# drepion43/distributed-mnist-BNNs

Measured on AMD Instinct MI355X. Metric: train samples/sec (node) + binary GEMM TOPS, higher is better.
Workload: dtype fp4/fp6/int8 MFMA (ternary operands as FP4 e2m1, fp32 operands as 4 FP6 e2m3 digit planes with E8M0 block scales + an FP4 residual plane on the dX operands (backward: within 2^-19 / 2^-22 of the block maximum) or 3 int8 digit planes (first layer); fp32 accumulate, fp32 I/O); 1 GPU; wide binarized MLP 784-8192x3-10 (BASELINE config 5); model=wide, global_batch=65536, per_gpu_batch=65536, seq_len=1, parallelism=dp1, backend=fp4, exchange=False, hip_graph=False

## Files before the change

distributed-mnist-bnns_amd/bnn_amd/functional.py:

```python
import collections
import contextlib
import ctypes
import itertools
import os

import torch

from . import _lib as L

__all__ = [
    "KernelTimer", "timing", "sign", "sign_pack", "sign_pack_bits", "quant_rows", "quant_cols_t", "gemm_i8", "gemm_xnor",
    "quant6_rows", "quant6_cols_t", "gemm_fp6", "set_digit_gemm",
    "binary_linear", "binary_conv2d", "hardtanh_backward", "adam_clamp_", "adam_clamp_pack_", "packed_weight",
    "sgd_clamp_", "sgd_clamp_multi_", "sgd_clamp_pack_",
    "invalidate_packed", "batch_norm_hardtanh",
    "bn_hardtanh_binary_linear", "batch_norm2d_hardtanh_pool", "dropout_batch_norm_hardtanh", "dropout_mask",
    "BinaryLinearFunction", "BinaryConv2dFunction",
]

ALIGN = 64


class KernelTimer:

# ... 879 lines not shown

def _const_vec(val, n, device):
    key = (float(val), int(n), str(device))
    t = _CONST.get(key)
    if t is None:
        t = torch.full((n,), float(val), dtype=torch.float32, device=device)
        _CONST[key] = t
    return t


PIX_STATS = os.environ.get("BNN_PIX_STATS", "1") != "0"
_FSTATS_ATTR = "_bnn_fstats"
PIX_STATS_USES = 0


def _pixels_fwd_with_stats(q, wq, M, N, K, bscale, bias, R, s0):
    chunk = int(L.lib().bnn_gemm_i8_bnstats_chunk(M, N))
    rows = (M + chunk - 1) // chunk
    part = torch.empty((2, rows, N), dtype=torch.float64, device=q.device)
    y = torch.empty((M, N), dtype=torch.float32, device=q.device)
    Kp = q.shape[1]
    assert wq.shape[1] == Kp and Kp % ALIGN == 0
    name = f"{gemm_kernel_name(1, 1, M, N, Kp)} [pixels]" if _TIMER is not None else ""
    with _timed(name, 2.0 * M * N * K, M * Kp + N * Kp + 4 * M * N):
        L.call("bnn_gemm_i8_affine_bnstats", q, Kp, wq, Kp, bscale, bias, R, float(s0), y, N, M, N, Kp, part, rows,
               L.stream())
    setattr(y, _FSTATS_ATTR, (part, rows, chunk, M, N, "pixels", 0.0, 0))
    return y


S20 = os.environ.get("BNN_S20", "1") != "0"
S20_HANDOFFS = 0


def _s20_of(x):
    z = getattr(x, _PREACT_ATTR, None)
    return z.args if z is not None and z.kind == "s20" else None


def dense_preact(z):
    d = getattr(z, _PREACT_ATTR, None)
    return z if d is None else d.dense()


def _pixels_fwd_s20(q, wq, M, N, K, a, bias, R, s0):
    chunk = int(L.lib().bnn_gemm_i8_bnstats_chunk(M, N))
    rows = (M + chunk - 1) // chunk
    dev = q.device
    part = torch.empty((2, rows, N), dtype=torch.float64, device=dev)
    lo = torch.empty((M, N), dtype=torch.int16, device=dev)
    hi = torch.empty((M, N // 2), dtype=torch.uint8, device=dev)
    Kp = q.shape[1]
    assert wq.shape[1] == Kp and Kp % ALIGN == 0
    name = f"{gemm_kernel_name(1, 1, M, N, Kp)} [pixels s20]" if _TIMER is not None else ""
    with _timed(name, 2.0 * M * N * K, M * Kp + N * Kp + 2.5 * M * N):
        L.call("bnn_gemm_i8_affine_bnstats_s20", q, Kp, wq, Kp, R, float(s0), K, lo, hi, N, M, N, Kp, part, rows,
               _const_vec(a, N, dev), bias, L.stream())
    y = _preact_carrier(PreAct("s20", lo, hi, bias, float(a)))
    setattr(y, _FSTATS_ATTR, (part, rows, chunk, M, N, "pixels", 0.0, 0))
    return y


def _fstats_of(z, M, C, drop=(0.0, 0)):
    fs = getattr(z, _FSTATS_ATTR, None)
    if fs is None or fs[3] != M or fs[4] != C or z._version != 0:
        return None
    p, seed = float(drop[0]), int(drop[1])
    if fs[6] != p or (p > 0 and fs[7] != seed):
        return None
    return fs


FP4_STATS = os.environ.get("BNN_FP4_STATS", "1") != "0"
FP4_STATS_USES = 0


def _fp4_fwd_with_stats(q, wq, M, N, k_true, bias, zbias, chunk, i16, drop=(0.0, 0)):
    Kb = q.shape[1]
    assert wq.shape[1] == Kb and Kb % ALIGN == 0
    rows = (M + chunk - 1) // chunk
    part = torch.empty((2, rows, N), dtype=torch.float64, device=q.device)
    C = torch.empty((M, N), dtype=torch.int16 if i16 else torch.float32, device=q.device)
    name = (gemm_kernel_name(0, 0, M, N, Kb) + (" [i16]" if i16 else "")) if _TIMER is not None else ""
    with _timed(name, 2.0 * M * N * k_true, (M + N) * Kb + (2 if i16 else 4) * M * N):
        L.call("bnn_gemm_fp4_bnstats", q, Kb, wq, Kb, None if i16 else bias, None if i16 else C, C if i16 else None, N,
               zbias, M, N, Kb, float(drop[0]), int(drop[1]), part, rows, L.stream())
    return C, (part, rows, chunk, M, N, "fp4", float(drop[0]), int(drop[1]))


class BinaryLinearPixelsFunction(torch.autograd.Function):

    @staticmethod
    def forward(ctx, u, weight, bias, a, s0, cache=False, emit_s20=False):
        _check(u, dtype=torch.uint8)
        _check(weight, bias)
        M, K = u.shape
        N = weight.shape[0]
        ctx.dims = (M, K, N)
        ctx.has_bias = bias is not None
        ctx.a, ctx.s0 = a, s0
        need_dw = ctx.needs_input_grad[1]
        q, qt = pixels_pack(u, want_q=M > 0, want_qt=need_dw and M > 0)
        if M == 0:
            ctx.save_for_backward(None)
            return torch.empty((0, N), dtype=torch.float32, device=u.device)
        wq, _ = packed_weight(weight, "i8", True, False, cache)
        R = row_sums(wq, K)
# ... 173 lines not shown
        L.call("bnn_hinge_bwd", x, y, t, M, C, float(margin), int(bool(squared)), go, dx, L.stream())
    return dx


def hinge_loss_ok(input, target):
    if not (torch.is_tensor(input) and torch.is_tensor(target) and input.is_cuda and input.dim() == 2
            and input.dtype == torch.float32 and input.shape[0] > 0 and target.device == input.device
            and bool(L.lib().bnn_hinge_ok(input.shape[1]))):
        return False
    if target.dtype == torch.int64:
        return target.dim() == 1 and target.shape[0] == input.shape[0]
    return target.dtype == torch.float32 and target.shape == input.shape and not target.requires_grad


def hinge_loss(input, target, margin=1.0, squared=False):
    _check(input)
    if not hinge_loss_ok(input, target):
        raise ValueError("bnn_amd: hinge_loss needs float32 CUDA [M, C] logits (M > 0, C in 2, 10, 16, 32, 64) and "
                         f"int64 [M] labels or a float32 target of the same shape without grad; got "
                         f"{tuple(input.shape)} {input.dtype} and {tuple(target.shape)} {target.dtype}")
    return HingeLossFunction.apply(input, target, float(margin), bool(squared))


def _pair_same(v, what):
    if isinstance(v, (tuple, list)):
        if len(set(v)) != 1:
            raise NotImplementedError(f"bnn_amd: asymmetric {what} {v} is not supported")
        return int(v[0])
    return int(v)


C1BN = os.environ.get("BNN_C1BN", "1") != "0"
_C1BN_WANT = "_bnn_c1bn_consumer"
_C1BN_ATTR = "_bnn_c1bn"
C1BN_HANDOFFS = 0


_C1bnHandoff = collections.namedtuple("_C1bnHandoff", "zq zb zf dyp mean invstd gw gb sg sgx inv_n ht")


def _c1bn_take(dy):
    ent = _take(dy, _C1BN_ATTR, stale="stale conv1 / BatchNorm2d hand-off",
                lost="a conv gradient placeholder lost its BatchNorm2d hand-off")
    return None if ent is None else _C1bnHandoff(*ent)


_CONV_C1F = [os.environ.get("BNN_CONV_C1F")]
if os.environ.get("BNN_FP6_PERS") is not None:
    L.call("bnn_gemm_fp6_set_persistent", int(os.environ["BNN_FP6_PERS"] != "0"))
if os.environ.get("BNN_FP6_HALF") is not None:
    L.call("bnn_gemm_fp6_set_half", int(os.environ["BNN_FP6_HALF"]), 0.0)
if os.environ.get("BNN_PIX_TILE") is not None:
    L.call("bnn_gemm_i8_bnstats_set_tile", int(os.environ["BNN_PIX_TILE"]))
if os.environ.get("BNN_HEAD_RED_COLS") is not None:
    L.call("bnn_bn_set_head_reduce_cols", int(os.environ["BNN_HEAD_RED_COLS"]))


def _conv_env():
    if _CONV_C1F[0] is not None:
        L.call("bnn_conv_set_c1_filter", int(_CONV_C1F[0] != "0"))
        _CONV_C1F[0] = None


ZQ = True
ZQ_HANDOFFS = 0


def _zq_fmt(x, binarize_input, stride, dilation, groups, C, KH, KW, H, W, pad, N, Co):
    if not (ZQ and binarize_input and stride == 1 and dilation == 1 and groups == 1 and pad <= min(KH, KW) - 1):
        return 0
    if not (C == 1 and KW <= 8) and not (C % 16 == 0 and C <= 64):
        return 0
    fmt = 2 if C * KH * KW <= 32767 else 0
    if fmt and not L.lib().bnn_conv2d_fwd_q_ok(fmt, N, C, H, W, Co, KH, KW, stride, pad, dilation, groups):
        return 0
    return fmt


def conv_out_hw(H, W, KH, KW, stride, padding, dilation):
    eh, ew = dilation * (KH - 1) + 1, dilation * (KW - 1) + 1
    if eh > H + 2 * padding or ew > W + 2 * padding:
        raise ValueError(f"conv2d: dilated kernel ({eh} x {ew}) can't be greater than the padded input "
                         f"({H + 2 * padding} x {W + 2 * padding})")
    return (H + 2 * padding - eh) // stride + 1, (W + 2 * padding - ew) // stride + 1


class BinaryConv2dFunction(torch.autograd.Function):
    @staticmethod
    def forward(ctx, x, weight, bias, binarize_input, stride, padding, dilation, groups, emit_compact=False,
                stochastic=None):
        _check(x, weight, bias)
        OH, OW = conv_out_hw(x.shape[2], x.shape[3], weight.shape[2], weight.shape[3], stride, padding, dilation)
        _conv_env()
        x = _c2d(x)
        if stochastic is not None and binarize_input:
            x = binarize_stochastic(x, stochastic)
        w = _c2d(weight.detach())
        N, C, H, W = x.shape
        Co, _, KH, KW = w.shape
        b = bias.detach() if bias is not None else None
        ctx.empty = N == 0
        ctx.save_for_backward(x, w)
        ctx.conf = (binarize_input, stride, padding, dilation, groups)
        ctx.has_bias = bias is not None
        zf = _zq_fmt(x, binarize_input, stride, dilation, groups, C, KH, KW, H, W, padding, N, Co) if emit_compact else 0
        if zf and N > 0 and Co <= 64 and (OH * OW) % 4 == 0 and OH % 2 == 0 and OW % 2 == 0:
# ... 867 lines not shown
```

distributed-mnist-bnns_amd/csrc/bnn_gemm.hip:

```cpp
#include <algorithm>
#include <type_traits>

#include "bnn_common.h"

namespace bnn {
namespace {

constexpr int BK = 64;

struct GemmParams {
  const int8_t* A;
  const int8_t* B;
  int64_t lda, ldb, a_plane, b_plane;
  const float* a_scale;
  const float* b_scale;
  const float* bias;
  float* C;
  int64_t ldc;
  int M, N, K;
  int gm, gn;
  const int64_t* row_off;
  const int64_t* col_off;
  double off_mul;
  int16_t* C16 = nullptr;
// ... 718 lines not shown
            const uint32_t lo = (uint32_t)(uint16_t)(int16_t)v.x | ((uint32_t)(uint16_t)(int16_t)v.y << 16);
            const uint32_t hi = (uint32_t)(uint16_t)(int16_t)v.z | ((uint32_t)(uint16_t)(int16_t)v.w << 16);
            out_store2u(d16, lo, hi);
          } else {
            const float vs[4] = {v.x, v.y, v.z, v.w};
#pragma unroll
            for (int j = 0; j < 4; ++j)
              if (c0 + j < p.N) d16[j] = (int16_t)vs[j];
          }
          continue;
        }
        float* dst = p.C + (int64_t)row * p.ldc + c0;
#ifdef GEMM_DIAG_NOSTORE
        if (p.M > 0) continue;
#endif
        if (vec_ok && c0 + 3 < p.N) {
          out_store4f(dst, v);
        } else {
          const float vs[4] = {v.x, v.y, v.z, v.w};
#pragma unroll
          for (int j = 0; j < 4; ++j)
            if (c0 + j < p.N) dst[j] = vs[j];
        }
      }
      asm volatile("s_waitcnt lgkmcnt(0)" ::: "memory");
    }
  }
}

template <int DA, int DB, int WAVES_M, int WAVES_N, int WM, int WN, int STAGES, int BKT, int IL = 0,
          int DIAG = 0, int S16 = 0, int BST = 0>
__global__ __launch_bounds__(64 * WAVES_M * WAVES_N) void gemm_i8_v2_k(GemmParams p) {
  gemm_v2_body<DA, DB, WAVES_M, WAVES_N, WM, WN, STAGES, BKT, IL, DIAG, 0, S16, BST>(p);
}

template <int WAVES_M, int WAVES_N, int WM, int WN, int STAGES, int BKT, int IL = 0, int S16 = 0, int BST = 0>
__global__ __launch_bounds__(64 * WAVES_M * WAVES_N) void gemm_fp4_k(GemmParams p) {
  gemm_v2_body<1, 1, WAVES_M, WAVES_N, WM, WN, STAGES, BKT, IL, 0, 1, S16, BST>(p);
}

template <int WAVES_M, int WAVES_N, int WM, int WN, int STAGES, int BKT, int IL = 0, int S16 = 0, int BST = 0>
__global__ __launch_bounds__(64 * WAVES_M * WAVES_N, 2) void gemm_fp4_h_k(GemmParams p) {
  gemm_v2_body<1, 1, WAVES_M, WAVES_N, WM, WN, STAGES, BKT, IL, 0, 1, S16, BST>(p);
}

template <int WAVES_M, int WAVES_N, int WM, int WN, int STAGES, int BKT, int IL = 0, int S16 = 0>
__global__ __launch_bounds__(64 * WAVES_M * WAVES_N) void gemm_fp4_bnsign_k(GemmParams p) {
  gemm_v2_body<1, 1, WAVES_M, WAVES_N, WM, WN, STAGES, BKT, IL, 0, 1, S16, 0, 1>(p);
}

template <int WAVES_M, int WAVES_N, int WM, int WN, int STAGES, int BKT>
__global__ __launch_bounds__(64 * WAVES_M * WAVES_N) void gemm_i8_bnsign_k(GemmParams p) {
  gemm_v2_body<1, 1, WAVES_M, WAVES_N, WM, WN, STAGES, BKT, 0, 0, 0, 0, 0, 1>(p);
}

template <int F4, int WAVES_M, int WAVES_N, int WM, int WN, int STAGES, int BKT, int IL = 0, int S16 = 0>
int launch_bnsign(GemmParams p, hipStream_t s) {
  constexpr int BM = WAVES_M * WM * 32, BN = WAVES_N * WN * 32;
  p.gm = (p.M + BM - 1) / BM;
  p.gn = (p.N + BN - 1) / BN;
  const int64_t covered = (int64_t)p.gn * BN / 2;
  if (covered < p.ldq4) {
    const hipError_t e = hipMemset2DAsync(p.Q4 + covered, (size_t)p.ldq4, 0, (size_t)(p.ldq4 - covered), (size_t)p.M, s);
    if (e != hipSuccess) {
      set_error("bnn_gemm_bnsign: clearing the pad failed: %s", hipGetErrorString(e));
      return (int)e;
    }
  }
  const dim3 grid((unsigned)((int64_t)p.gm * p.gn)), block(64 * WAVES_M * WAVES_N);
  if constexpr (F4) {
    hipLaunchKernelGGL((gemm_fp4_bnsign_k<WAVES_M, WAVES_N, WM, WN, STAGES, BKT, IL, S16>), grid, block, 0, s, p);
    return check_launch("bnn_gemm_fp4_bnsign");
  } else {
    static_assert(IL == 0 && S16 == 0, "int8 BN-sign form: the 32x32 BK=64 kernels");
    hipLaunchKernelGGL((gemm_i8_bnsign_k<WAVES_M, WAVES_N, WM, WN, STAGES, BKT>), grid, block, 0, s, p);
    return check_launch("bnn_gemm_i8_affine_bnsign");
  }
}

template <int WAVES_M, int WAVES_N, int WM, int WN, int STAGES, int BKT, int IL = 0, int S16 = 0, int BST = 0>
int launch_fp4h(GemmParams p, hipStream_t s) {
  constexpr int BM = WAVES_M * WM * 32, BN = WAVES_N * WN * 32;
  p.gm = (p.M + BM - 1) / BM;
  p.gn = (p.N + BN - 1) / BN;
  hipLaunchKernelGGL((gemm_fp4_h_k<WAVES_M, WAVES_N, WM, WN, STAGES, BKT, IL, S16, BST>),
                     dim3((unsigned)((int64_t)p.gm * p.gn)), dim3(64 * WAVES_M * WAVES_N), 0, s, p);
  return check_launch("bnn_gemm_fp4");
}

template <int DA, int DB, int WAVES_M, int WAVES_N, int WM, int WN, int STAGES, int BKT, int IL = 0,
          int DIAG = 0, int F4 = 0, int S16 = 0, int BST = 0>
int launch_v2(GemmParams p, hipStream_t s) {
  constexpr int BM = WAVES_M * WM * 32, BN = WAVES_N * WN * 32;
  p.gm = (p.M + BM - 1) / BM;
  p.gn = (p.N + BN - 1) / BN;
  const int64_t nblk = (int64_t)p.gm * p.gn;
  if constexpr (F4) {
    static_assert(DA == 1 && DB == 1 && DIAG == 0, "FP4 form");
    hipLaunchKernelGGL((gemm_fp4_k<WAVES_M, WAVES_N, WM, WN, STAGES, BKT, IL, S16, BST>), dim3((unsigned)nblk),
                       dim3(64 * WAVES_M * WAVES_N), 0, s, p);
    return check_launch("bnn_gemm_fp4");
  } else {
    hipLaunchKernelGGL((gemm_i8_v2_k<DA, DB, WAVES_M, WAVES_N, WM, WN, STAGES, BKT, IL, DIAG, S16, BST>),
                       dim3((unsigned)nblk), dim3(64 * WAVES_M * WAVES_N), 0, s, p);
    return check_launch("bnn_gemm_i8");
  }
// ... 80 lines not shown
    id = base + g_variant;
    alt = base + 1;
  } else if (a_digits == 1) {
    const bool big = ((M + 255) / 256) * ((N + 255) / 256) >= 512;
    id = big ? 9 : 1;
    alt = big ? 2 : 1;
  } else if (b_digits == 1) {
    const bool big = ((M + 127) / 128) * ((N + 255) / 256) >= 256;
    id = big ? 18 : 13;
    alt = big ? 15 : 13;
  } else {
    id = 22;
    alt = 22;
  }
  const Variant* v = find_variant(id);
  if (v == nullptr) v = find_variant(base + 1);
  if (K % v->bk != 0) v = find_variant(alt);
  return v;
}

}
}

using namespace bnn;

BNN_API int bnn_gemm_i8_affine(const int8_t* A, int64_t lda, int64_t a_plane, int32_t a_digits,
                               const int8_t* B, int64_t ldb, int64_t b_plane, int32_t b_digits,
                               const float* a_scale, const float* b_scale, const float* bias,
                               const int64_t* row_off, const int64_t* col_off, double off_mul, float* C,
                               int64_t ldc, int64_t M, int64_t N, int64_t K, void* stream) {
  const bool cfg_ok = (a_digits == 1 && b_digits == 1) || (a_digits == 3 && b_digits == 1) ||
                      (a_digits == 3 && b_digits == 3);
  if (!A || !B || !C || !cfg_ok || M < 0 || N < 0 || K <= 0 || K % BK != 0 || lda < K || ldb < K ||
      lda % 16 != 0 || ldb % 16 != 0 || ldc < N || !aligned16(A) || !aligned16(B) ||
      M > 0x7fffffff || N > 0x7fffffff || K > 0x7fffffff ||
      (a_digits > 1 && (a_plane < M * lda || a_plane % 16 != 0)) ||
      (b_digits > 1 && (b_plane < N * ldb || b_plane % 16 != 0))) {
    set_error("bnn_gemm_i8_affine: bad arguments (M=%lld N=%lld K=%lld lda=%lld ldb=%lld digits=%d,%d; "
              "K must be a positive multiple of 64)",
              (long long)M, (long long)N, (long long)K, (long long)lda, (long long)ldb, a_digits,
              b_digits);
    return kErrInval;
  }
  if (M == 0 || N == 0) return 0;
  GemmParams p{A, B, lda, ldb, a_plane, b_plane, a_scale, b_scale, bias, C, ldc,
               (int)M, (int)N, (int)K, 0, 0, row_off, col_off, off_mul};
  p.raster = g_raster;
  if (lda * 256 >= (1LL << 31) || ldb * 256 >= (1LL << 31))
    return find_variant(a_digits == 1 ? 0 : (b_digits == 1 ? 10 : 20))->fn(p, reinterpret_cast<hipStream_t>(stream));
  return pick_kernel(a_digits, b_digits, M, N, K)->fn(p, reinterpret_cast<hipStream_t>(stream));
}

static int g_i8_bnstats_tile = 0;

static const Variant* i8_bnstats_variant(int64_t M, int64_t N) {
  const bool big = ((M + 255) / 256) * ((N + 255) / 256) >= 512;
  if (g_i8_bnstats_tile != 0) return find_variant(g_i8_bnstats_tile == 2 ? 2 : 1);
  return find_variant(big ? 2 : 1);
}

BNN_API int32_t bnn_gemm_i8_bnstats_set_tile(int32_t tile) {
  if (tile < 0) return g_i8_bnstats_tile;
  if (tile > 2) return kErrInval;
  g_i8_bnstats_tile = tile;
  return 0;
}

BNN_API int64_t bnn_gemm_i8_bnstats_chunk(int64_t M, int64_t N) {
  return i8_bnstats_variant(M, N)->id == 2 ? 128 : 64;
}

static bool i8_bnstats_shape_ok(int64_t M, int64_t N, int64_t K, int64_t lda, int64_t ldb) {
  return M > 0 && N > 0 && K > 0 && K % BK == 0 && lda >= K && ldb >= K && lda % 16 == 0 && ldb % 16 == 0 &&
         M <= 0x7fffffff && N <= 0x7fffffff && K <= 0x7fffffff && lda * 256 < (1LL << 31) &&
         ldb * 256 < (1LL << 31) &&
         (double)M * (128.0 * K) * (128.0 * K) < 9007199254740992.0;
}

BNN_API int bnn_gemm_i8_bnstats_ok(int64_t M, int64_t N, int64_t K, int64_t lda, int64_t ldb) {
  return i8_bnstats_shape_ok(M, N, K, lda, ldb) ? 1 : 0;
}

BNN_API int bnn_gemm_i8_affine_bnstats(const int8_t* A, int64_t lda, const int8_t* B, int64_t ldb,
                                       const float* b_scale, const float* bias, const int64_t* col_off,
                                       double off_mul, float* C, int64_t ldc, int64_t M, int64_t N, int64_t K,
                                       double* stat, int64_t stat_rows, void* stream) {
  const int64_t chunk = M > 0 ? bnn_gemm_i8_bnstats_chunk(M, N) : 1;
  if (!A || !B || !C || !stat || !i8_bnstats_shape_ok(M, N, K, lda, ldb) || ldc < N || !aligned16(A) ||
      !aligned16(B) || stat_rows != (M + chunk - 1) / chunk) {
    set_error("bnn_gemm_i8_affine_bnstats: bad arguments (M=%lld N=%lld K=%lld stat_rows=%lld; want %lld)",
              (long long)M, (long long)N, (long long)K, (long long)stat_rows, (long long)((M + chunk - 1) / chunk));
    return kErrInval;
  }
  GemmParams p{A, B, lda, ldb, 0, 0, nullptr, b_scale, bias, C, ldc,
               (int)M, (int)N, (int)K, 0, 0, nullptr, col_off, off_mul};
  p.stat = stat;
  p.stat_rows = stat_rows;
  hipStream_t st = reinterpret_cast<hipStream_t>(stream);
  return i8_bnstats_variant(M, N)->id == 2 ? launch_v2<1, 1, 2, 4, 4, 2, 3, 64, 0, 0, 0, 0, 1>(p, st)
                                           : launch_v2<1, 1, 2, 2, 2, 2, 3, 64, 0, 0, 0, 0, 1>(p, st);
}

BNN_API int bnn_gemm_i8_s20_ok(int64_t M, int64_t N, int64_t K, int64_t k_true, double s0) {
  return (N % 4 == 0 && s0 == (double)(int64_t)s0 && k_true > 0 && k_true <= K &&
          (double)k_true * (128.0 + fabs(s0)) < 524288.0)
             ? 1
             : 0;
}

BNN_API int bnn_gemm_i8_affine_bnstats_s20(const int8_t* A, int64_t lda, const int8_t* B, int64_t ldb,
                                           const int64_t* col_off, double off_mul, int64_t k_true, int16_t* Slo,
                                           uint8_t* Shi, int64_t ldc, int64_t M, int64_t N, int64_t K, double* stat,
                                           int64_t stat_rows, const float* b_scale, const float* bias, void* stream) {
  const int64_t chunk = M > 0 ? bnn_gemm_i8_bnstats_chunk(M, N) : 1;
  if (!A || !B || !Slo || !Shi || !col_off || !stat || !i8_bnstats_shape_ok(M, N, K, lda, ldb) || ldc < N ||
      ldc % 4 != 0 || !aligned16(A) || !aligned16(B) || (reinterpret_cast<uintptr_t>(Slo) & 7) != 0 ||
      (reinterpret_cast<uintptr_t>(Shi) & 1) != 0 || !bnn_gemm_i8_s20_ok(M, N, K, k_true, off_mul) ||
      stat_rows != (M + chunk - 1) / chunk) {
    set_error("bnn_gemm_i8_affine_bnstats_s20: bad arguments (M=%lld N=%lld K=%lld k_true=%lld off_mul=%g "
              "stat_rows=%lld)", (long long)M, (long long)N, (long long)K, (long long)k_true, off_mul,
              (long long)stat_rows);
    return kErrInval;
  }
  GemmParams p{A, B, lda, ldb, 0, 0, nullptr, b_scale, bias, nullptr, ldc,
               (int)M, (int)N, (int)K, 0, 0, nullptr, col_off, off_mul};
  p.stat = stat;
  p.stat_rows = stat_rows;
  p.S20lo = Slo;
  p.S20hi = Shi;
  hipStream_t st = reinterpret_cast<hipStream_t>(stream);
  return i8_bnstats_variant(M, N)->id == 2 ? launch_v2<1, 1, 2, 4, 4, 2, 3, 64, 0, 0, 0, 0, 1>(p, st)
                                           : launch_v2<1, 1, 2, 2, 2, 2, 3, 64, 0, 0, 0, 0, 1>(p, st);
}

BNN_API int bnn_gemm_i8(const int8_t* A, int64_t lda, int64_t a_plane, int32_t a_digits,
                        const int8_t* B, int64_t ldb, int64_t b_plane, int32_t b_digits,
                        const float* a_scale, const float* b_scale, const float* bias, float* C,
                        int64_t ldc, int64_t M, int64_t N, int64_t K, void* stream) {
  return bnn_gemm_i8_affine(A, lda, a_plane, a_digits, B, ldb, b_plane, b_digits, a_scale, b_scale, bias,
                            nullptr, nullptr, 0.0, C, ldc, M, N, K, stream);
}

BNN_API int bnn_gemm_fp4(const uint8_t* A, int64_t lda, const uint8_t* B, int64_t ldb, const float* bias,
                         float* C, int64_t ldc, int64_t M, int64_t N, int64_t K, void* stream) {
  if (!A || !B || !C || M < 0 || N < 0 || K <= 0 || K % BK != 0 || lda < K || ldb < K || lda % 16 != 0 ||
      ldb % 16 != 0 || ldc < N || !aligned16(A) || !aligned16(B) || M > 0x7fffffff || N > 0x7fffffff ||
      K > 0x7fffffff || lda * 256 >= (1LL << 31) || ldb * 256 >= (1LL << 31)) {
    set_error("bnn_gemm_fp4: bad arguments (M=%lld N=%lld K=%lld bytes; K must be a positive multiple of 64 "
              "and below 2^23 bytes)",
              (long long)M, (long long)N, (long long)K);
    return kErrInval;
  }
  if (M == 0 || N == 0) return 0;
  GemmParams p{reinterpret_cast<const int8_t*>(A), reinterpret_cast<const int8_t*>(B), lda, ldb, 0, 0,
               nullptr, nullptr, bias, C, ldc, (int)M, (int)N, (int)K, 0, 0, nullptr, nullptr, 0.0};
  return pick_kernel(0, 0, M, N, K)->fn(p, reinterpret_cast<hipStream_t>(stream));
}

BNN_API int bnn_gemm_fp4_i16(const uint8_t* A, int64_t lda, const uint8_t* B, int64_t ldb, int16_t* C16,
                             int64_t ldc, int64_t M, int64_t N, int64_t K, void* stream) {
  if (!C16 || ldc % 4 != 0 || (reinterpret_cast<uintptr_t>(C16) & 7) != 0 || 2 * K > 32767) {
    set_error("bnn_gemm_fp4_i16: bad arguments (ldc=%lld, K=%lld bytes; ldc %% 4 == 0, 8-B aligned output, "
              "2K <= 32767)", (long long)ldc, (long long)K);
    return kErrInval;
  }
  if (!A || !B || M < 0 || N < 0 || K <= 0 || K % BK != 0 || lda < K || ldb < K || lda % 16 != 0 ||
      ldb % 16 != 0 || ldc < N || !aligned16(A) || !aligned16(B) || M > 0x7fffffff || N > 0x7fffffff ||
      lda * 256 >= (1LL << 31) || ldb * 256 >= (1LL << 31)) {
    set_error("bnn_gemm_fp4_i16: bad arguments (M=%lld N=%lld K=%lld bytes)", (long long)M, (long long)N,
              (long long)K);
    return kErrInval;
  }
  if (M == 0 || N == 0) return 0;
  GemmParams p{reinterpret_cast<const int8_t*>(A), reinterpret_cast<const int8_t*>(B), lda, ldb, 0, 0,
               nullptr, nullptr, nullptr, nullptr, ldc, (int)M, (int)N, (int)K, 0, 0, nullptr, nullptr, 0.0, C16};
  return pick_kernel(0, 0, M, N, K)->fn(p, reinterpret_cast<hipStream_t>(stream));
}

BNN_API int64_t bnn_gemm_fp4_bnstats_chunk(int64_t M, int64_t N, int64_t K) {
  const int id = pick_kernel(0, 0, M, N, K)->id;
  return id == 31 ? 64 : (id == 36 ? 128 : 0);
}

BNN_API int bnn_gemm_fp4_bnstats(const uint8_t* A, int64_t lda, const uint8_t* B, int64_t ldb, const float* bias,
                                 float* C, int16_t* C16, int64_t ldc, const float* zbias, int64_t M, int64_t N,
// ... 94 lines not shown
```

include/bnn.h:

```cpp
#ifndef BNN_H_
#define BNN_H_

#include <stdint.h>

#ifdef __cplusplus
extern "C" {
#endif

#define BNN_EINVAL (-1)

typedef void* bnn_stream_t;

int bnn_version(void);
const char* bnn_last_error(void);

int bnn_sign_pack_i8(const float* x, int64_t M, int64_t K, int64_t ldx, int8_t* q, int64_t ldq,
                     int8_t* qt, int64_t ldqt, bnn_stream_t stream);

int bnn_sign_pack_fp4(const float* x, int64_t M, int64_t K, int64_t ldx, uint8_t* q4, int64_t ldq4,
                      int8_t* qt, int64_t ldqt, int32_t qt_fmt, bnn_stream_t stream);

int bnn_sign_f32(const float* x, float* y, int64_t n, bnn_stream_t stream);

int bnn_sign_pack_fp4_out(const float* x, int64_t M, int64_t K, uint8_t* q4, int64_t ldq4, int8_t* qt,
                          int64_t ldqt, int32_t qt_fmt, float* sout, bnn_stream_t stream);

int bnn_binarize_stoch_f32(const float* x, float* y, int64_t n, uint64_t seed, bnn_stream_t stream);
int bnn_stoch_pack_i8(const float* x, int64_t M, int64_t K, int64_t ldx, int8_t* q, int64_t ldq, int8_t* qt,
                      int64_t ldqt, uint64_t seed, bnn_stream_t stream);
int bnn_stoch_pack_fp4(const float* x, int64_t M, int64_t K, int64_t ldx, uint8_t* q4, int64_t ldq4, int8_t* qt,
                       int64_t ldqt, int32_t qt_fmt, uint64_t seed, int32_t force, bnn_stream_t stream);
int bnn_stoch_pack_fp4_out(const float* x, int64_t M, int64_t K, uint8_t* q4, int64_t ldq4, int8_t* qt,
                           int64_t ldqt, int32_t qt_fmt, float* sout, uint64_t seed, int32_t force,
                           bnn_stream_t stream);

int bnn_sign_pack_bits(const float* x, int64_t M, int64_t K, int64_t ldx, uint32_t* sbits,
                       uint32_t* nzbits, int64_t ldw, bnn_stream_t stream);

int bnn_quant_rows(const float* x, int64_t M, int64_t K, int64_t ldx, int8_t* digits, int64_t ldq,
                   int64_t plane, float* scale, bnn_stream_t stream);

int64_t bnn_quant_cols_workspace(int64_t M, int64_t N);
int bnn_quant_cols_t(const float* x, int64_t M, int64_t N, int64_t ldx, int8_t* digits_t,
                     int64_t ldqt, int64_t plane, float* scale, float* colsum, void* work,
                     bnn_stream_t stream);
int bnn_quant_cols_t_dsum(const float* x, int64_t M, int64_t N, int64_t ldx, int8_t* digits_t,
                          int64_t ldqt, int64_t plane, float* scale, float* colsum, int64_t* dsum,
                          void* work, bnn_stream_t stream);

int bnn_gemm_i8(const int8_t* A, int64_t lda, int64_t a_plane, int32_t a_digits,
                const int8_t* B, int64_t ldb, int64_t b_plane, int32_t b_digits,
                const float* a_scale, const float* b_scale, const float* bias, float* C,
                int64_t ldc, int64_t M, int64_t N, int64_t K, bnn_stream_t stream);

int bnn_gemm_i8_affine(const int8_t* A, int64_t lda, int64_t a_plane, int32_t a_digits,
                       const int8_t* B, int64_t ldb, int64_t b_plane, int32_t b_digits,
                       const float* a_scale, const float* b_scale, const float* bias,
                       const int64_t* row_off, const int64_t* col_off, double off_mul, float* C,
                       int64_t ldc, int64_t M, int64_t N, int64_t K, bnn_stream_t stream);

int64_t bnn_gemm_i8_bnstats_chunk(int64_t M, int64_t N);

int64_t bnn_gemm_fp4_bnstats_chunk(int64_t M, int64_t N, int64_t K);
int bnn_gemm_fp4_bnstats(const uint8_t* A, int64_t lda, const uint8_t* B, int64_t ldb, const float* bias,
                         float* C, int16_t* C16, int64_t ldc, const float* zbias, int64_t M, int64_t N, int64_t K,
                         float drop_p, uint64_t drop_seed, double* stat, int64_t stat_rows, bnn_stream_t stream);
int bnn_gemm_i8_bnstats_set_tile(int32_t tile);
int bnn_gemm_i8_affine_bnstats(const int8_t* A, int64_t lda, const int8_t* B, int64_t ldb,
                               const float* b_scale, const float* bias, const int64_t* col_off,
                               double off_mul, float* C, int64_t ldc, int64_t M, int64_t N, int64_t K,
                               double* stat, int64_t stat_rows, bnn_stream_t stream);
int bnn_gemm_i8_bnstats_ok(int64_t M, int64_t N, int64_t K, int64_t lda, int64_t ldb);

int bnn_gemm_i8_s20_ok(int64_t M, int64_t N, int64_t K, int64_t k_true, double s0);
int bnn_gemm_i8_affine_bnstats_s20(const int8_t* A, int64_t lda, const int8_t* B, int64_t ldb,
                                   const int64_t* col_off, double off_mul, int64_t k_true, int16_t* Slo,
                                   uint8_t* Shi, int64_t ldc, int64_t M, int64_t N, int64_t K, double* stat,
                                   int64_t stat_rows, const float* b_scale, const float* bias, bnn_stream_t stream);

int bnn_unit_to_pixels(const float* x, int64_t n, uint8_t* u, int32_t* bad, bnn_stream_t stream);
int bnn_pixels_pack(const uint8_t* x, int64_t M, int64_t K, int64_t ldx, int8_t* q, int64_t ldq,
                    int8_t* qt, int64_t ldqt, bnn_stream_t stream);
int bnn_row_sums(const int8_t* q, int64_t N, int64_t K, int64_t ldq, int64_t* out, bnn_stream_t stream);

int bnn_gemm_fp4(const uint8_t* A, int64_t lda, const uint8_t* B, int64_t ldb, const float* bias,
                 float* C, int64_t ldc, int64_t M, int64_t N, int64_t K, bnn_stream_t stream);

int bnn_gemm_fp4_i16(const uint8_t* A, int64_t lda, const uint8_t* B, int64_t ldb, int16_t* C16, int64_t ldc,
                     int64_t M, int64_t N, int64_t K, bnn_stream_t stream);

int bnn_gemm_fp4_bnsign(const uint8_t* A, int64_t lda, const uint8_t* B, int64_t ldb, const float* bias,
                        const float* mean, const float* invstd, const float* gamma, const float* beta,
                        uint8_t* q4, int64_t ldq4, int64_t M, int64_t N, int64_t K, bnn_stream_t stream);
int bnn_gemm_i8_affine_bnsign(const int8_t* A, int64_t lda, const int8_t* B, int64_t ldb,
                              const float* b_scale, const float* bias, const int64_t* col_off, double off_mul,
                              const float* mean, const float* invstd, const float* gamma, const float* beta,
                              uint8_t* q4, int64_t ldq4, int64_t M, int64_t N, int64_t K, bnn_stream_t stream);

int bnn_gemm_set_variant(int32_t variant);
int bnn_gemm_set_raster(int32_t raster);
const char* bnn_gemm_i8_kernel(int32_t a_digits, int32_t b_digits, int64_t M, int64_t N,
                               int64_t K);

int64_t bnn_quant6_scale_rows(int64_t rows);
int bnn_quant6_rows(const float* x, int64_t M, int64_t K, int64_t ldx, int64_t Kp, uint8_t* lo, uint8_t* hi,
                    uint8_t* sc, uint8_t* res , bnn_stream_t stream);
int64_t bnn_quant6_cols_workspace(int64_t M, int64_t N);
int bnn_quant6_cols_t(const float* x, int64_t M, int64_t N, int64_t ldx, int64_t Mp, uint8_t* lo, uint8_t* hi,
                      uint8_t* sc, float* colsum, void* work, bnn_stream_t stream);
int bnn_gemm_fp6(const uint8_t* alo, const uint8_t* ahi, const uint8_t* asc, int64_t asc_rows, const uint8_t* ares,
                 const uint8_t* b, int64_t ldb, const float* bias, float* C, int64_t ldc, int64_t M, int64_t N,
                 int64_t K, bnn_stream_t stream);
int64_t bnn_gemm_fp6_workspace(int64_t M, int64_t N, int64_t K);
int bnn_gemm_fp6_ws(const uint8_t* alo, const uint8_t* ahi, const uint8_t* asc, int64_t asc_rows,
                    const uint8_t* ares, const uint8_t* b, int64_t ldb, const float* bias, float* C, int64_t ldc,
                    int64_t M, int64_t N, int64_t K, void* work, int64_t work_bytes, bnn_stream_t stream);
int64_t bnn_fp4_panel_bytes(int64_t N, int64_t Kp);
int bnn_fp4_panelize(const uint8_t* b, int64_t N, int64_t ldb, int64_t Kp, uint8_t* panels, bnn_stream_t stream);
int bnn_gemm_fp6_panel_ws(const uint8_t* alo, const uint8_t* ahi, const uint8_t* asc, int64_t asc_rows,
                          const uint8_t* ares, const uint8_t* bpanels, int64_t bks, const float* bias, float* C,
                          int64_t ldc, int64_t M, int64_t N, int64_t K, void* work, int64_t work_bytes,
                          bnn_stream_t stream);
int64_t bnn_gemm_fp6_bnstats_rows(int64_t M);
int bnn_gemm_fp6_bnstats(const uint8_t* alo, const uint8_t* ahi, const uint8_t* asc, int64_t asc_rows,
                         const uint8_t* ares, const uint8_t* bpanels, int64_t bks, float* C, int64_t ldc, int64_t M,
                         int64_t N, int64_t K,
                         const void* x, const float* xbias, int32_t x_i16, const float* mean, const float* mean_lo,
// ... 299 lines not shown
```

Before: 1.528 million samples/s.

## Add dedicated u8-pixel s20 first-layer GEMM kernel with LDS-patch packed epilogue

Adds a specialized int8 MFMA kernel for the first-layer pixel GEMM that writes the split 20-bit output (int16 low plane plus 4-bit high nibbles). The epilogue stages accumulators through a swizzled LDS patch, packs them, and uses DPP lane moves so each row segment goes out as wide 16-byte stores. It also fuses the BN statistics reduction. The new default (form 2) runs a smaller one-wave-row tile with 2 stages and occupancy 3, replacing the generic v2 kernel for large shapes. This adds code complexity and changes tile shape and occupancy, which may or may not suit the MI355X.

```diff
diff --git a/distributed-mnist-bnns_amd/bnn_amd/functional.py b/distributed-mnist-bnns_amd/bnn_amd/functional.py
--- a/distributed-mnist-bnns_amd/bnn_amd/functional.py
+++ b/distributed-mnist-bnns_amd/bnn_amd/functional.py
@@ -955,7 +955,7 @@
     hi = torch.empty((M, N // 2), dtype=torch.uint8, device=dev)
     Kp = q.shape[1]
     assert wq.shape[1] == Kp and Kp % ALIGN == 0
-    name = f"{gemm_kernel_name(1, 1, M, N, Kp)} [pixels s20]" if _TIMER is not None else ""
+    name = f"{L.lib().bnn_gemm_i8_s20_kernel(M, N).decode()} [pixels s20]" if _TIMER is not None else ""
     with _timed(name, 2.0 * M * N * K, M * Kp + N * Kp + 2.5 * M * N):
         L.call("bnn_gemm_i8_affine_bnstats_s20", q, Kp, wq, Kp, R, float(s0), K, lo, hi, N, M, N, Kp, part, rows,
                _const_vec(a, N, dev), bias, L.stream())
@@ -1235,6 +1235,8 @@
     L.call("bnn_gemm_fp6_set_half", int(os.environ["BNN_FP6_HALF"]), 0.0)
 if os.environ.get("BNN_PIX_TILE") is not None:
     L.call("bnn_gemm_i8_bnstats_set_tile", int(os.environ["BNN_PIX_TILE"]))
+if os.environ.get("BNN_PIX_S20_FORM") is not None:
+    L.call("bnn_gemm_i8_s20_set_form", int(os.environ["BNN_PIX_S20_FORM"]))
 if os.environ.get("BNN_HEAD_RED_COLS") is not None:
     L.call("bnn_bn_set_head_reduce_cols", int(os.environ["BNN_HEAD_RED_COLS"]))
 
diff --git a/distributed-mnist-bnns_amd/csrc/bnn_gemm.hip b/distributed-mnist-bnns_amd/csrc/bnn_gemm.hip
--- a/distributed-mnist-bnns_amd/csrc/bnn_gemm.hip
+++ b/distributed-mnist-bnns_amd/csrc/bnn_gemm.hip
@@ -794,6 +794,194 @@
 template <int WAVES_M, int WAVES_N, int WM, int WN, int STAGES, int BKT>
 __global__ __launch_bounds__(64 * WAVES_M * WAVES_N) void gemm_i8_bnsign_k(GemmParams p) {
   gemm_v2_body<1, 1, WAVES_M, WAVES_N, WM, WN, STAGES, BKT, 0, 0, 0, 0, 0, 1>(p);
+}
+
+__device__ __forceinline__ void out_store4u(void* p, uint32_t a, uint32_t b, uint32_t c, uint32_t d) {
+  if (BNN_NT_STORES) __builtin_nontemporal_store(v4u{a, b, c, d}, reinterpret_cast<v4u*>(p));
+  else *reinterpret_cast<uint4*>(p) = make_uint4(a, b, c, d);
+}
+
+template <int DA, int DB, int WAVES_M, int WAVES_N, int WM, int WN, int STAGES, int BKT, int OCC = 2>
+__global__ __launch_bounds__(64 * WAVES_M * WAVES_N, OCC) void gemm_i8_px_s20_k(GemmParams p) {
+  static_assert(DA == 1 && DB == 1 && WN == 2 && BKT == 64, "the u8-pixel (1,1) form, patch pairs, BK = 64");
+  constexpr int NW = WAVES_M * WAVES_N;
+  constexpr int BM = WAVES_M * WM * 32, BN = WAVES_N * WN * 32;
+  constexpr int A_ST = BM * BKT, B_ST = BN * BKT, ST = A_ST + B_ST;
+  constexpr int RPI = 1024 / BKT, CPR = BKT / 16;
+  constexpr int IA = BM / RPI, IB = BN / RPI;
+  static_assert(IA % NW == 0 && IB % NW == 0, "glds instructions must split evenly over waves");
+  constexpr int PER_WAVE = (IA + IB) / NW;
+  constexpr int KSTEPS = BKT / 32;
+  constexpr int PATCH = 32 * 64;
+  static_assert(NW * PATCH * 4 <= STAGES * ST, "the epilogue's patches reuse the operand ring");
+  __shared__ __attribute__((aligned(16))) char smem[STAGES * ST];
+
+  const int lane = threadIdx.x & 63, wave = wave_id();
+  const int wm = wave / WAVES_N, wn = wave % WAVES_N;
+  int tm, tn;
+  tile_of(blockIdx.x, p.gm, p.gn, tm, tn);
+  const int m0 = tm * BM, n0 = tn * BN;
+
+  auto swz = [](int row) { return (row >> 2) & 3; };
+  const int srow = lane / CPR, sslot = lane % CPR;
+  const int lim_a = p.M - 1 - m0, lim_b = p.N - 1 - n0;
+  auto stage = [&](int kt, int buf) {
+    char* sA = smem + buf * ST;
+    char* sB = sA + A_ST;
+#pragma unroll
+    for (int i = 0; i < IA / NW; ++i) {
+      const int jr = wave + i * NW;
+      const int lrow = jr * RPI + srow;
+      const uint32_t voff = (uint32_t)min(lrow, lim_a) * (uint32_t)p.lda + 16u * (uint32_t)(sslot ^ swz(lrow));
+      glds16_s(p.A + (int64_t)m0 * p.lda + (int64_t)kt * BKT, voff, sA + jr * 1024);
+    }
+#pragma unroll
+    for (int i = 0; i < IB / NW; ++i) {
+      const int jr = wave + i * NW;
+      const int lrow = jr * RPI + srow;
+      const uint32_t voff = (uint32_t)min(lrow, lim_b) * (uint32_t)p.ldb + 16u * (uint32_t)(sslot ^ swz(lrow));
+      glds16_s(p.B + (int64_t)n0 * p.ldb + (int64_t)kt * BKT, voff, sB + jr * 1024);
+    }
+  };
+
+  v16i acc[WM][WN];
+#pragma unroll
+  for (int t = 0; t < WM; ++t)
+#pragma unroll
+    for (int u = 0; u < WN; ++u) acc[t][u] = v16i{0};
+
+  const int r = lane & 31, h = lane >> 5, sw = swz(r);
+  const int nk = p.K / BKT;
+#pragma unroll
+  for (int s = 0; s < STAGES - 1; ++s)
+    if (s < nk) stage(s, s);
+  for (int kt = 0; kt < nk; ++kt) {
+    wait_stages<PER_WAVE, STAGES - 2>(min(STAGES - 2, nk - 1 - kt));
+    block_barrier();
+    if (kt + STAGES - 1 < nk) stage(kt + STAGES - 1, (kt + STAGES - 1) % STAGES);
+    const char* sA = smem + (kt % STAGES) * ST;
+    const char* sB = sA + A_ST;
+    v4i a[2][WM], b[2][WN];
+    auto load_frags = [&](int ks, v4i (&fa)[WM], v4i (&fb)[WN]) {
+      const int off = 16 * ((2 * ks + h) ^ sw);
+#pragma unroll
+      for (int t = 0; t < WM; ++t)
+        fa[t] = *reinterpret_cast<const v4i*>(sA + (wm * WM * 32 + t * 32 + r) * BKT + off);
+#pragma unroll
+      for (int u = 0; u < WN; ++u)
+        fb[u] = *reinterpret_cast<const v4i*>(sB + (wn * WN * 32 + u * 32 + r) * BKT + off);
+    };
+    load_frags(0, a[0], b[0]);
+#pragma unroll
+    for (int ks = 0; ks < KSTEPS; ++ks) {
+      if (ks + 1 < KSTEPS) load_frags(ks + 1, a[(ks + 1) & 1], b[(ks + 1) & 1]);
+#pragma unroll
+      for (int t = 0; t < WM; ++t)
+#pragma unroll
+        for (int u = 0; u < WN; ++u)
+          acc[t][u] = __builtin_amdgcn_mfma_i32_32x32x32_i8(a[ks & 1][t], b[ks & 1][u], acc[t][u], 0, 0, 0);
+    }
+  }
+  wait_vmcnt_c<0>();
+  block_barrier();
+
+  const int cr0 = m0 + wm * WM * 32;
+  const int cnt = min(WM * 32, p.M - cr0);
+  const bool full = cr0 + WM * 32 <= p.M;
+  const int lim = p.M - cr0 - 4 * h;
+  const int64_t chunk = (int64_t)tm * WAVES_M + wm, RN = p.stat_rows * (int64_t)p.N;
+  int icoff[WN];
+#pragma unroll
+  for (int u = 0; u < WN; ++u) {
+    const int col = n0 + wn * WN * 32 + u * 32 + r;
+    const bool cin = col < p.N;
+    const double coff = cin ? (double)p.col_off[col] * p.off_mul : 0.0;
+    icoff[u] = (int)coff;
+    int i1 = 0;
+    double d2 = 0.0;
+#pragma unroll
+    for (int t = 0; t < WM; ++t)
+#pragma unroll
+      for (int i = 0; i < 16; ++i) {
+        const int v = (full || (t * 32 + (i & 3) + 8 * (i >> 2)) < lim) ? acc[t][u][i] : 0;
+        const double d = (double)v;
+        i1 += v;
+        d2 = fma(d, d, d2);
+      }
+    i1 += __shfl_xor(i1, 32, 64);
+    d2 += __shfl_xor(d2, 32, 64);
+    if (h == 0 && cnt > 0 && cin) {
+      const double s1 = (double)i1, s2 = d2;
+      const double a = p.b_scale ? (double)p.b_scale[col] : 1.0;
+      const double b = p.bias ? (double)p.bias[col] : 0.0;
+      p.stat[chunk * p.N + col] = a * (s1 + cnt * coff) + cnt * b;
+      const double m2 = s2 - s1 * s1 / cnt;
+      p.stat[RN + chunk * p.N + col] = a * a * (m2 > 0.0 ? m2 : 0.0);
+    }
+  }
+
+  int* patch = reinterpret_cast<int*>(smem) + wave * PATCH;
+  const int tcol0 = n0 + wn * WN * 32;
+  const int lc8 = lane & 7;
+  const int c0 = tcol0 + 8 * lc8;
+  const bool lo16 = ((p.ldc & 7) == 0) && ((reinterpret_cast<uintptr_t>(p.S20lo) & 15) == 0);
+  const bool hi16 = ((p.ldc & 31) == 0) && ((reinterpret_cast<uintptr_t>(p.S20hi) & 15) == 0) &&
+                    tcol0 + 32 * (lc8 >> 2) + 32 <= p.N;
+#pragma unroll
+  for (int t = 0; t < WM; ++t) {
+    const int trow0 = m0 + wm * WM * 32 + t * 32;
+#pragma unroll
+    for (int u = 0; u < WN; ++u)
+#pragma unroll
+      for (int i = 0; i < 16; ++i) {
+        const int lr = (i & 3) + 8 * (i >> 2) + 4 * h;
+        const int lc = u * 32 + r;
+        patch[lr * 64 + ((((lc >> 2) ^ (i & 1)) << 2) | (lc & 3))] = acc[t][u][i] + icoff[u];
+      }
+    asm volatile("s_waitcnt lgkmcnt(0)" ::: "memory");
+#pragma unroll
+    for (int ps = 0; ps < 4; ++ps) {
+      const int lr = (lane >> 3) + 8 * ps, odd = lr & 1;
+      const v4i x = *reinterpret_cast<const v4i*>(patch + lr * 64 + ((2 * lc8 + odd) << 2));
+      const v4i y = *reinterpret_cast<const v4i*>(patch + lr * 64 + ((2 * lc8 + 1 - odd) << 2));
+      const uint32_t s[8] = {(uint32_t)x.x, (uint32_t)x.y, (uint32_t)x.z, (uint32_t)x.w,
+                             (uint32_t)y.x, (uint32_t)y.y, (uint32_t)y.z, (uint32_t)y.w};
+      uint32_t lo[4], hi = 0u;
+#pragma unroll
+      for (int j = 0; j < 4; ++j) lo[j] = (s[2 * j] & 0xFFFFu) | (s[2 * j + 1] << 16);
+#pragma unroll
+      for (int j = 0; j < 8; ++j) hi |= ((s[j] >> 16) & 0xFu) << (4 * j);
+      const uint32_t h1 = (uint32_t)__builtin_amdgcn_mov_dpp((int)hi, 0x55, 0xF, 0xF, true);
+      const uint32_t h2 = (uint32_t)__builtin_amdgcn_mov_dpp((int)hi, 0xAA, 0xF, 0xF, true);
+      const uint32_t h3 = (uint32_t)__builtin_amdgcn_mov_dpp((int)hi, 0xFF, 0xF, 0xF, true);
+      const int row = trow0 + lr;
+      if (row >= p.M) continue;
+      const int64_t o = (int64_t)row * p.ldc + c0;
+      if (lo16 && c0 + 8 <= p.N) {
+        out_store4u(p.S20lo + o, lo[0], lo[1], lo[2], lo[3]);
+      } else {
+        if (c0 < p.N) out_store2u(p.S20lo + o, lo[0], lo[1]);
+        if (c0 + 4 < p.N) out_store2u(p.S20lo + o + 4, lo[2], lo[3]);
+      }
+      if (hi16) {
+        if ((lane & 3) == 0) out_store4u(p.S20hi + (o >> 1), hi, h1, h2, h3);
+      } else {
+        if (c0 < p.N) *reinterpret_cast<uint16_t*>(p.S20hi + (o >> 1)) = (uint16_t)hi;
+        if (c0 + 4 < p.N) *reinterpret_cast<uint16_t*>(p.S20hi + (o >> 1) + 2) = (uint16_t)(hi >> 16);
+      }
+    }
+    asm volatile("s_waitcnt lgkmcnt(0)" ::: "memory");
+  }
+}
+
+template <int WAVES_M, int STAGES = 3, int OCC = 2>
+int launch_px_s20(GemmParams p, hipStream_t s) {
+  constexpr int BM = WAVES_M * 128, BN = 256;
+  p.gm = (p.M + BM - 1) / BM;
+  p.gn = (p.N + BN - 1) / BN;
+  hipLaunchKernelGGL((gemm_i8_px_s20_k<1, 1, WAVES_M, 4, 4, 2, STAGES, 64, OCC>), dim3((unsigned)((int64_t)p.gm * p.gn)),
+                     dim3(64 * WAVES_M * 4), 0, s, p);
+  return check_launch("bnn_gemm_i8_affine_bnstats_s20");
 }
 
 template <int F4, int WAVES_M, int WAVES_N, int WM, int WN, int STAGES, int BKT, int IL = 0, int S16 = 0>
@@ -980,6 +1168,7 @@
 }
 
 static int g_i8_bnstats_tile = 0;
+static int g_px_s20_form = 2;
 
 static const Variant* i8_bnstats_variant(int64_t M, int64_t N) {
   const bool big = ((M + 255) / 256) * ((N + 255) / 256) >= 512;
@@ -1057,8 +1246,27 @@
   p.S20lo = Slo;
   p.S20hi = Shi;
   hipStream_t st = reinterpret_cast<hipStream_t>(stream);
-  return i8_bnstats_variant(M, N)->id == 2 ? launch_v2<1, 1, 2, 4, 4, 2, 3, 64, 0, 0, 0, 0, 1>(p, st)
-                                           : launch_v2<1, 1, 2, 2, 2, 2, 3, 64, 0, 0, 0, 0, 1>(p, st);
+  if (i8_bnstats_variant(M, N)->id != 2) return launch_v2<1, 1, 2, 2, 2, 2, 3, 64, 0, 0, 0, 0, 1>(p, st);
+  if (g_px_s20_form == 1) return launch_px_s20<2>(p, st);
+  if (g_px_s20_form == 2) return launch_px_s20<1, 2, 3>(p, st);
+  return launch_v2<1, 1, 2, 4, 4, 2, 3, 64, 0, 0, 0, 0, 1>(p, st);
+}
+
+BNN_API int32_t bnn_gemm_i8_s20_set_form(int32_t form) {
+  if (form < 0) return g_px_s20_form;
+  if (form > 2) {
+    set_error("bnn_gemm_i8_s20_set_form: form %d (0 .. 2)", (int)form);
+    return kErrInval;
+  }
+  g_px_s20_form = form;
+  return 0;
+}
+
+BNN_API const char* bnn_gemm_i8_s20_kernel(int64_t M, int64_t N) {
+  if (i8_bnstats_variant(M, N)->id != 2) return "gemm_i8_v2_k<1, 1, 2, 2, 2, 2, 3, 64, 0, 0, 0, 1>";
+  if (g_px_s20_form == 1) return "gemm_i8_px_s20_k<1, 1, 2, 4, 4, 2, 3, 64, 2>";
+  if (g_px_s20_form == 2) return "gemm_i8_px_s20_k<1, 1, 1, 4, 4, 2, 2, 64, 3>";
+  return "gemm_i8_v2_k<1, 1, 2, 4, 4, 2, 3, 64, 0, 0, 0, 1>";
 }
 
 BNN_API int bnn_gemm_i8(const int8_t* A, int64_t lda, int64_t a_plane, int32_t a_digits,
diff --git a/include/bnn.h b/include/bnn.h
--- a/include/bnn.h
+++ b/include/bnn.h
@@ -73,6 +73,8 @@
 int bnn_gemm_i8_bnstats_ok(int64_t M, int64_t N, int64_t K, int64_t lda, int64_t ldb);
 
 int bnn_gemm_i8_s20_ok(int64_t M, int64_t N, int64_t K, int64_t k_true, double s0);
+int bnn_gemm_i8_s20_set_form(int32_t form);
+const char* bnn_gemm_i8_s20_kernel(int64_t M, int64_t N);
 int bnn_gemm_i8_affine_bnstats_s20(const int8_t* A, int64_t lda, const int8_t* B, int64_t ldb,
                                    const int64_t* col_off, double off_mul, int64_t k_true, int16_t* Slo,
                                    uint8_t* Shi, int64_t ldc, int64_t M, int64_t N, int64_t K, double* stat,
```

Result: no change. 1.543 million samples/s (median of 6 runs) (+0.9%).
